# jzbontar/mc-cnn

Measured on AMD Instinct MI355X. Metric: Mega-pixel-disparities/sec (cost-vol+CBCA+SGM) + end-to-end disp ms/pair, higher is better.
Workload: dtype f32; 1 GPU; KITTI 2012 fast, 370x1226 disp_max=228; H=370, W=1226, disp_max=228, feature_channels=64, params=kitti_fast, parallelism=one pair per GPU

## Files before the change

### mc-cnn_amd/csrc/api.hip

```cpp
#include "cbca_common.h"

#include <stdarg.h>
#include <algorithm>
#include <map>
#include <mutex>
#include <vector>

namespace mc {

int fill_nan(float *p, int64_t n, hipStream_t st);
int scale(const float *in, float *out, int64_t n, float s, hipStream_t st);
int transpose(const float *in, float *out, int64_t R, int64_t Cn, int64_t ldin, int64_t ldout, float s, hipStream_t st, int nt = -1);
int fix_border(float *vol, int D, int H, int W, int n, int direction, hipStream_t st);
int argmin_dhw(const float *vol, float *out, int D, int H, int W, int base1, hipStream_t st);
int outlier_detection(const float *d0, const float *d1, float *outlier, int H, int W, int disp_max, hipStream_t st);
int interpolate_occlusion(const float *d0, const float *outlier, float *out, int H, int W, hipStream_t st);
int interpolate_mismatch(const float *d0, const float *outlier, float *out, int H, int W, hipStream_t st);
int subpixel(const float *d0, const float *vol, float *out, int D, int H, int W, int64_t sd, int64_t sp, hipStream_t st);
int median2d(const float *img, float *out, int H, int W, int k, hipStream_t st);
int mean2d(const float *img, const float *kernel, float *out, int H, int W, int ks, float alpha2, hipStream_t st);
int normalize_forward(const float *in, float *norm, float *out, int N, int C, int H, int W, hipStream_t st);
int stereo_join_dhw(const float *fL, const float *fR, float *volL, float *volR, int C, int D, int H, int W, hipStream_t st);
int stereo_join_hwd(const float *fL, const float *fR, float *volL, float *volR, int C, int D, int ds, int H, int W, int n,
                    hipStream_t st);
// ... 17 lines not shown
                  hipStream_t st, bool two_pass = false, float cost_limit = 0);
int cbca_lean2x(const void *packed, const void *plan, size_t plan_bytes, const float *vin, float *vout, int D, int H, int W, int direction,
                int route, hipStream_t st, const CbcaCfg &cfg);
int cbca_lean(const void *packed, const void *plan, size_t plan_bytes, const float *vin, float *vout, int D, int H, int W, int direction,
              int route, hipStream_t st, const CbcaCfg &cfg);
size_t conv3x3_workspace_bytes(int Cin, int Cout);
int conv3x3(const float *in, const float *w, const float *bias, float *out, int N, int Cin, int Cout, int H, int W, int relu,
            void *workspace, hipStream_t st);
size_t fc_workspace_bytes(int C, int n_hidden, int H, int W);
int fc_stack(const float *featL, const float *featR, int C, int H, int W, int D, const float *const *weights,
             const float *const *biases, int n_layers, float *volL, float *volR, void *workspace, hipStream_t st);
size_t sgm_maps_bytes(int H, int W);
int sgm_prep(const float *x0, const float *x1, void *maps, int H, int W, float tau_so, hipStream_t st);
int sgm_contract_violations(const float *vol, int H, int W, int D, unsigned *count, hipStream_t st);
int sgm_sweeps(const float *const C[2], float *const out[2], float *const out2[2], float *const disp[2],
               const int direction[2], int nvol, int H, int W, int D, int ds, const void *maps, float pi1, float pi2,
               float alpha1, float q1, float q2, bool fused, unsigned drop_final, hipStream_t st);

static thread_local char g_err[512] = "";

void set_error(const char *fmt, ...)
{
	va_list ap;
	va_start(ap, fmt);
	vsnprintf(g_err, sizeof(g_err), fmt, ap);
	va_end(ap);
}

int check_launch(const char *what)
{
	const hipError_t e = hipPeekAtLastError();
	if (e != hipSuccess) {
		(void)hipGetLastError();
		set_error("%s: %s", what, hipGetErrorString(e));
		return (int)e;
	}
	return 0;
}

static bool dims_ok(int D, int H, int W) { return D >= 1 && H >= 1 && W >= 1 && (int64_t)D * H * W < ((int64_t)1 << 40); }

static void gaussian_fill(double sigma, float *k)
{
	const int kr = (int)ceil(sigma * 3);
	const int ks = kr * 2 + 1;
	for (int i = 1; i <= ks; ++i) {
		for (int j = 1; j <= ks; ++j) {
			const double y = (i - 1) - kr;
			const double x = (j - 1) - kr;
			k[(size_t)(i - 1) * ks + (j - 1)] = (float)exp(-(x * x + y * y) / (2 * sigma * sigma));
		}
	}
}
struct GaussianK { const float *data; size_t n; };
static int gaussian_cached(double sigma, GaussianK &out)
{
	static std::mutex mu;
	static std::map<double, GaussianK> cache;
	std::lock_guard<std::mutex> lk(mu);
	auto it = cache.find(sigma);
	if (it != cache.end()) { out = it->second; return 0; }
	const int kr = (int)ceil(sigma * 3);
	const int ks = kr * 2 + 1;
	float *k = nullptr;
	const hipError_t e = hipHostMalloc((void **)&k, (size_t)ks * ks * sizeof(float), hipHostMallocDefault);
	if (e != hipSuccess) {
		set_error("gaussian: hipHostMalloc: %s", hipGetErrorString(e));
		return (int)e;
	}
	gaussian_fill(sigma, k);
	out = GaussianK{k, (size_t)ks * ks};
	cache[sigma] = out;
	return 0;
}

static inline size_t align_up(size_t v, size_t a) { return (v + a - 1) / a * a; }

static inline bool packed_dims_ok(int H, int W)
{
	return (int64_t)H * W < ((int64_t)1 << 29) - 4096 && H < (1 << 23) - 64 && W < (1 << 23) - 256;
}

static int cbca_by_arms(const void *packed, const float *vin, float *vout, int D, int H, int W, int direction, int max_arm, hipStream_t st,
                        const CbcaCfg &cfg = CbcaCfg())
{
	if (max_arm >= 0 && max_arm <= 4) return cbca_tiles(packed, vin, vout, D, H, W, direction, 4, -1, st, cfg);
	if (cfg.planned) {
		int rc = cbca_tiles(packed, vin, vout, D, H, W, direction, 13, CR_PLANNED_TILE13, st, cfg);
		if (rc || cfg.lean_two_pass) return rc;
		return cbca_strips(packed, vin, vout, D, H, W, direction, CR_STRIP_IF_LIST, st, cfg);
	}
	int rc = cbca_tiles(packed, vin, vout, D, H, W, direction, 4, CR_TILE4, st, cfg);
	if (rc) return rc;
	if (max_arm < 0 || max_arm <= 13) {
		rc = cbca_tiles(packed, vin, vout, D, H, W, direction, 13, CR_TILE13, st, cfg);
		if (rc) return rc;
	}
	if (cfg.lean) {
		if (!cfg.lean_two_pass) {
			rc = cbca_lean(packed, cfg.plan, cfg.plan_bytes, vin, vout, D, H, W, direction, CR_STRIP, st, cfg);
			if (rc) return rc;
		}
		return cbca_strips(packed, vin, vout, D, H, W, direction, CR_STRIP_IF_NO_LIST, st, cfg);
	}
	return cbca_strips(packed, vin, vout, D, H, W, direction, max_arm > 13 ? CR_STRIP_OR_TILE13 : CR_STRIP, st, cfg);
}

struct Plan {
	int Dp;
	size_t maps, arms, pack, vol, img, gk;
	size_t cplan;
	int nplan;
	size_t total;
};

struct StageCounts { int cbca1, sgm, cbca2; bool active_after; };
static StageCounts stage_counts(const mc_params *p)
{
	StageCounts c;
	bool sm_active = p->sm_terminate != MC_SM_CNN;
	c.cbca1 = (sm_active && p->sm_skip != MC_SKIP_CBCA) ? p->cbca_i1 : 0;
	sm_active = sm_active && p->sm_terminate != MC_SM_CBCA1;
	c.sgm = (sm_active && p->sm_skip != MC_SKIP_SGM) ? p->sgm_i : 0;
	sm_active = sm_active && p->sm_terminate != MC_SM_SGM;
	c.cbca2 = (sm_active && p->sm_skip != MC_SKIP_CBCA) ? p->cbca_i2 : 0;
// ... 41 lines not shown
	{
		for (int i = 0; i < MC_N_STAGES; ++i) out[i] = 0;
		if (!on || ev.empty()) return;
		(void)hipEventSynchronize(ev.back());
		for (size_t i = 1; i < ev.size(); ++i) {
			float ms = 0;
			(void)hipEventElapsedTime(&ms, ev[i - 1], ev[i]);
			if (tag[i] >= 0 && tag[i] < MC_N_STAGES) out[tag[i]] += ms;
		}
		for (auto e : ev) (void)hipEventDestroy(e);
		ev.clear();
	}
};
enum { ST_PREP = MC_STAGE_PREP, ST_JOIN = MC_STAGE_JOIN, ST_CBCA = MC_STAGE_CBCA, ST_LAYOUT = MC_STAGE_LAYOUT,
       ST_SGM = MC_STAGE_SGM, ST_ARGMIN = MC_STAGE_ARGMIN, ST_POST = MC_STAGE_POST };

static int predict_impl(const mc_params *p, const float *x0, const float *x1, const float *featL, const float *featR, int C,
                        const float *rawL, const float *rawR, int D, int H, int W, void *workspace, size_t workspace_bytes,
                        float *volL_out, float *volR_out, float *dispL0_out, float *dispR0_out, float *disp_out, hipStream_t st,
                        StageTimer &tm)
{
	MC_REQUIRE(p && x0 && x1 && disp_out && workspace, "mc_predict: null argument");
	MC_REQUIRE(dims_ok(D, H, W), "mc_predict: bad dims D=%d H=%d W=%d", D, H, W);
	MC_REQUIRE(D <= MC_SGM_MAX_D, "mc_predict: D=%d exceeds %d", D, MC_SGM_MAX_D);
	MC_REQUIRE((featL && featR && C >= 1) || (rawL && rawR), "mc_predict: need features or raw volumes");
	MC_REQUIRE(p->cbca_i1 >= 0 && p->cbca_i2 >= 0 && p->sgm_i >= 0, "mc_predict: negative iteration count");
	MC_REQUIRE(p->median_k % 2 == 1 && p->median_k <= 11, "mc_predict: median_k must be odd and <= 11");
	MC_REQUIRE(p->blur_sigma > 0, "mc_predict: blur_sigma must be > 0");
	MC_REQUIRE(p->sm_terminate >= 0 && p->sm_terminate <= MC_SM_BILATERAL && p->sm_skip >= 0 && p->sm_skip <= MC_SKIP_BILATERAL,
	           "mc_predict: bad sm_terminate / sm_skip");
	const bool from_feat = featL != nullptr;
	if (from_feat) MC_REQUIRE(p->border_n >= 0 && p->border_n < W, "mc_predict: border_n=%d out of range", p->border_n);
	if (from_feat) MC_REQUIRE(C <= MC_JOIN_MAX_C, "mc_predict: C=%d exceeds %d (adcensus.cu:1460)", C, MC_JOIN_MAX_C);
	const Plan pl = make_plan(p, D, H, W);
	MC_REQUIRE(workspace_bytes >= pl.total, "mc_predict: workspace %zu < %zu bytes", workspace_bytes, pl.total);
	MC_REQUIRE((uintptr_t)workspace % 256 == 0, "mc_predict: workspace must be 256-byte aligned");

	const int64_t HW = (int64_t)H * W;
	const int64_t V = (int64_t)D * HW;
	char *w = (char *)workspace;
	void *maps = w; w += pl.maps;
	float *x0c = (float *)w; float *x1c = x0c + 4 * HW; w += pl.arms;
	void *packed = w; w += pl.pack;
	float *bufA[2], *bufB[2];
	bufA[0] = (float *)w; w += pl.vol;
	bufA[1] = (float *)w; w += pl.vol;
	bufB[0] = (float *)w; w += pl.vol;
	bufB[1] = (float *)w; w += pl.vol;
	float *bufC[2];
	bufC[0] = (float *)w; w += pl.vol;
	bufC[1] = (float *)w; w += pl.vol;
	float *img[6];
	for (int i = 0; i < 6; ++i) { img[i] = (float *)w; w += pl.img; }
	float *gk = (float *)w; w += pl.gk;
	void *cplan[2] = {pl.cplan ? (void *)w : nullptr, (pl.cplan && pl.nplan > 1) ? (void *)(w + pl.cplan) : nullptr};
	int cplan_passes[2] = {0, 0};
	bool cplan_listed[2] = {false, false};
	const int Dp = pl.Dp;
	int rc;
#define RUN(call) do { rc = (call); if (rc) return rc; } while (0)

	const int direction[2] = {-1, 1};
	const StageCounts sc = stage_counts(p);
	const int n_cbca1 = sc.cbca1, n_sgm = sc.sgm, n_cbca2 = sc.cbca2;
	bool sm_active = sc.active_after;
	const bool use_cbca = (n_cbca1 + n_cbca2) > 0;
	tm.mark(-1);

	if (n_sgm > 0) RUN(sgm_prep(x0, x1, maps, H, W, p->tau_so, st));
	if (use_cbca) {
		RUN(cross(x0, x0c, H, W, p->L1, p->tau1, st));
		RUN(cross(x1, x1c, H, W, p->L1, p->tau1, st));
		RUN(cbca_pack(x0c, x1c, packed, H, W, st));
	}
	const int cbca_cap = p->L1 - 1;
	tm.mark(ST_PREP);

	const int ds = Dp;
	const float *cur[2];
	auto other = [&](int v) -> float * { return cur[v] == bufA[v] ? bufB[v] : bufA[v]; };
	bool hwd;
	const int nvol = (p->left_only && !p->lr_check && !volR_out && !dispR0_out) ? 1 : 2;
	auto cbca_iterations = [&](int n) -> int {
		const bool packed_ok = cbca_cap <= 254 && packed_dims_ok(H, W);
		for (int v = 0; v < nvol; ++v) {
			const bool planned = packed_ok && cplan[v] && cbca_cap > 4 && cbca_cap <= 13 && cbca_lean_fits(D, H, W, pl.cplan, true);
			if (planned && n > 0 && !cplan_listed[v]) {
				const int rc1 = cbca_classify(packed, cplan[v], pl.cplan, D, H, W, direction[v], CR_STRIP, 0, 0, st, true);
				if (rc1) return rc1;
				cplan_listed[v] = true;
			}
			for (int i = 0; i < n;) {
				float *dst = other(v);
				CbcaCfg cfg;
				cfg.plan = cplan[v];
				cfg.plan_bytes = pl.cplan;
				cfg.planned = planned;
				const bool two = planned && i + 1 < n;
				cfg.lean = cfg.lean_two_pass = two;
				float *mid = two ? bufC[v] : dst;
				for (int half = 0; half < (two ? 2 : 1); ++half) {
					cfg.plan_mode = cplan[v] ? (cplan_passes[v]++ == 0 ? 1 : 2) : 0;
					const float *src = half == 0 ? cur[v] : mid;
					float *to = (two && half == 0) ? mid : dst;
					const int rc2 = packed_ok ? cbca_by_arms(packed, src, to, D, H, W, direction[v], cbca_cap, st, cfg)
					                          : cbca(x0c, x1c, src, to, D, H, W, direction[v], st);
					if (rc2) return rc2;
// ... 72 lines not shown
	MC_REQUIRE(have_disp || !hwd, "mc_predict: an (H,W,D) volume without its arg-min");
	if (!have_disp) {
		for (int v = 0; v < nvol; ++v) RUN(argmin_dhw(cur[v], dispv[v], D, H, W, 0, st));
	}
	float *vout[2] = {volL_out, volR_out};
	for (int v = 0; v < nvol; ++v) {
		if (!vout[v]) continue;
		if (hwd) RUN(transpose(cur[v], vout[v], HW, D, ds, HW, 1.0f, st));
		else RUN(scale(cur[v], vout[v], V, 1.0f, st));
	}
	if (dispL0_out) RUN(scale(dispv[0], dispL0_out, HW, 1.0f, st));
	if (dispR0_out) RUN(scale(dispv[1], dispR0_out, HW, 1.0f, st));
	tm.mark(ST_ARGMIN);

	float *d = dispv[0];
	float *outl = img[4];
	int nfree = 0;
	float *freeimg[3] = {img[2], img[3], img[5]};
	auto next = [&]() -> float * {
		float *r = freeimg[nfree % 3];
		if (r == d) r = freeimg[++nfree % 3];
		++nfree;
		return r;
	};
	if (p->lr_check) {
		RUN(outlier_detection(d, dispv[1], outl, H, W, D, st));
		if (sm_active && p->sm_skip != MC_SKIP_OCCLUSION) {
			float *o = next();
			RUN(interpolate_occlusion(d, outl, o, H, W, st));
			d = o;
		}
		sm_active = sm_active && p->sm_terminate != MC_SM_OCCLUSION;
		if (sm_active && p->sm_skip != MC_SKIP_OCCLUSION) {
			float *o = next();
			RUN(interpolate_mismatch(d, outl, o, H, W, st));
			d = o;
		}
		sm_active = sm_active && p->sm_terminate != MC_SM_MISMATCH;
	}
	if (sm_active && p->sm_skip != MC_SKIP_SUBPIXEL) {
		float *o = next();
		if (hwd) RUN(subpixel(d, cur[0], o, D, H, W, 1, ds, st));
		else RUN(subpixel(d, cur[0], o, D, H, W, HW, 1, st));
		d = o;
	}
	sm_active = sm_active && p->sm_terminate != MC_SM_SUBPIXEL;
	if (sm_active && p->sm_skip != MC_SKIP_MEDIAN) {
		float *o = next();
		RUN(median2d(d, o, H, W, p->median_k, st));
		d = o;
	}
	sm_active = sm_active && p->sm_terminate != MC_SM_MEDIAN;
	if (sm_active && p->sm_skip != MC_SKIP_BILATERAL) {
		GaussianK k;
		RUN(gaussian_cached(p->blur_sigma, k));
		const int ks = 2 * (int)ceil(p->blur_sigma * 3) + 1;
		const hipError_t e = hipMemcpyAsync(gk, k.data, k.n * sizeof(float), hipMemcpyHostToDevice, st);
		if (e != hipSuccess) {
			set_error("mc_predict: kernel upload: %s", hipGetErrorString(e));
			return (int)e;
		}
		RUN(mean2d(d, gk, disp_out, H, W, ks, p->blur_t, st));
	} else {
		RUN(scale(d, disp_out, HW, 1.0f, st));
	}
	tm.mark(ST_POST);
#undef RUN
	return 0;
}

}

using namespace mc;

extern "C" {

int mc_version(void) { return MC_ABI_VERSION; }
const char *mc_last_error(void) { return g_err; }

int mc_fill_nan(float *p, int64_t n, void *stream)
{
	MC_REQUIRE(p || n == 0, "mc_fill_nan: null pointer");
	MC_REQUIRE(n >= 0, "mc_fill_nan: negative size");
	return fill_nan(p, n, as_stream(stream));
}

int mc_stereo_join(const float *featL, const float *featR, float *volL, float *volR, int C, int D, int H, int W, void *stream)
{
	MC_REQUIRE(featL && featR && volL && volR, "mc_stereo_join: null pointer");
	MC_REQUIRE(dims_ok(D, H, W) && C >= 1, "mc_stereo_join: bad dims C=%d D=%d H=%d W=%d", C, D, H, W);
	MC_REQUIRE(C <= MC_JOIN_MAX_C, "mc_stereo_join: C=%d exceeds %d (adcensus.cu:1460)", C, MC_JOIN_MAX_C);
	MC_REQUIRE(D <= 65535, "mc_stereo_join: D too large");
	return stereo_join_dhw(featL, featR, volL, volR, C, D, H, W, as_stream(stream));
}

int mc_ad(const float *x0, const float *x1, float *vol, int D, int H, int W, int direction, void *stream)
{
	MC_REQUIRE(x0 && x1 && vol, "mc_ad: null pointer");
	MC_REQUIRE(dims_ok(D, H, W), "mc_ad: bad dims");
	MC_REQUIRE(direction == -1 || direction == 1, "mc_ad: direction must be -1 or 1");
	MC_REQUIRE(D <= 65535, "mc_ad: D too large");
	return ad_tiled(x0, x1, vol, D, H, W, direction, as_stream(stream));
}

size_t mc_census_scratch_bytes(int Cimg, int H, int W)
{
	if (Cimg < 1 || H < 1 || W < 1) return 0;
	return census_scratch_bytes(Cimg, H, W);
}

int mc_census_ws(const float *x0, const float *x1, float *vol, int Cimg, int D, int H, int W, int direction, void *scratch,
                 size_t scratch_bytes, void *stream)
{
	MC_REQUIRE(x0 && x1 && vol && scratch, "mc_census_ws: null pointer");
	MC_REQUIRE(dims_ok(D, H, W) && Cimg >= 1 && D <= 65535, "mc_census_ws: bad dims");
// ... 369 lines not shown
```

### mc-cnn_amd/csrc/post.hip

```cpp
#include "mc_common.h"

namespace mc {


__global__ void __launch_bounds__(256) fill_nan_kernel(float *__restrict__ p, int64_t n)
{
	const float nanv = __builtin_nanf("");
	for (int64_t i = (int64_t)blockIdx.x * blockDim.x + threadIdx.x; i < n; i += (int64_t)gridDim.x * blockDim.x) p[i] = nanv;
}

__global__ void __launch_bounds__(256) scale_kernel(const float *__restrict__ in, float *__restrict__ out, int64_t n, float s)
{
	for (int64_t i = (int64_t)blockIdx.x * blockDim.x + threadIdx.x; i < n; i += (int64_t)gridDim.x * blockDim.x) out[i] = in[i] * s;
}
typedef float f4v_t __attribute__((ext_vector_type(4)));
__global__ void __launch_bounds__(256) scale4_kernel(const f4v_t *__restrict__ in, f4v_t *__restrict__ out, int64_t n4, float s)
{
	const int64_t i = (int64_t)blockIdx.x * 256 + threadIdx.x;
	if (i < n4) out[i] = in[i] * s;
}

template <bool NT>
__global__ void __launch_bounds__(256) transpose_kernel(const float *__restrict__ in, float *__restrict__ out, int64_t R,
                                                        int64_t Cn, int64_t ldin, int64_t ldout, float s)
// ... 198 lines not shown
	__shared__ int carry[256];
	__shared__ int first_valid;
	const int y = blockIdx.x, t = threadIdx.x;
	const int64_t row = (int64_t)y * W;
	const int seg = (W + 255) / 256;
	const int xa = t * seg, xb = min(W, xa + seg);
	if (t == 0) first_valid = W;
	int last = -1;
	for (int x = xa; x < xb; ++x)
		if (outlier[row + x] == 0) last = x;
	carry[t] = last;
	__syncthreads();
	if (last >= 0) {
		int f = -1;
		for (int x = xa; x < xb; ++x)
			if (outlier[row + x] == 0) { f = x; break; }
		atomicMin(&first_valid, f);
	}
	for (int off = 1; off < 256; off <<= 1) {
		const int o = t >= off ? carry[t - off] : -1;
		__syncthreads();
		carry[t] = max(carry[t], o);
		__syncthreads();
	}
	int lv = t > 0 ? carry[t - 1] : -1;
	const int fv = first_valid;
	for (int x = xa; x < xb; ++x) {
		const int64_t id = row + x;
		const float o = outlier[id];
		if (o == 0) lv = x;
		float r = d0[id];
		if (o == 1) {
			if (lv >= 0) r = d0[row + lv];
			else if (fv < W) r = d0[row + fv];
		}
		out[id] = r;
	}
}

int interpolate_occlusion(const float *d0, const float *outlier, float *out, int H, int W, hipStream_t st)
{
	hipLaunchKernelGGL(interp_occ_rows_kernel, dim3(H), dim3(256), 0, st, d0, outlier, out, W);
	return check_launch("interpolate_occlusion");
}

template <int K> __device__ __forceinline__ void ray_rank_step(float v, int inb, int &less, int &eq)
{
	const float ov = __uint_as_float(__builtin_amdgcn_update_dpp(0u, __float_as_uint(v), 0x120 + K, 0xf, 0xf, false));
	const int oin = __builtin_amdgcn_update_dpp(0, inb, 0x120 + K, 0xf, 0xf, false);
	less += (oin && ov < v) ? 1 : 0;
	eq += (oin && ov == v) ? 1 : 0;
}

#define MC_MIS_NU 4
__global__ void __launch_bounds__(256) interp_mis_rays_kernel(const float *__restrict__ d0, const float *__restrict__ outlier,
                                                              float *__restrict__ out, int size, int H, int W)
{
	const int t = blockIdx.x * blockDim.x + threadIdx.x;
	const int id = t >> 4;
	const int ray = (int)(threadIdx.x & 15);
	if (id >= size) return;
	const bool mis = outlier[id] == 2;
	if (!mis) {
		if (ray == 0) out[id] = d0[id];
		return;
	}
	const int hx[16] = {0, -1, -2, -2, -2, -2, -2, -1, 0, 1, 2, 2, 2, 2, 2, 1};
	const int hy[16] = {2, 2, 2, 1, 0, -1, -2, -2, -2, -2, -2, -1, 0, 1, 2, 2};
	const int x = id % W, y = id / W;
	const int sx = hx[ray], sy = hy[ray];
	const __amdgpu_buffer_rsrc_t ro = __builtin_amdgcn_make_buffer_rsrc((void *)outlier, 0, size * 4, 0x00020000);
	const __amdgpu_buffer_rsrc_t rd = __builtin_amdgcn_make_buffer_rsrc((void *)d0, 0, size * 4, 0x00020000);
	int X2 = 2 * x, Y2 = 2 * y;
	constexpr unsigned OOB = 0x80000000u;
	unsigned stop = OOB;
	for (bool go = true; go;) {
		unsigned off[MC_MIS_NU], o[MC_MIS_NU];
#pragma unroll
		for (int i = 0; i < MC_MIS_NU; ++i) {
			X2 += sx;
			Y2 += sy;
			const int xi = (X2 + 1 + (X2 >> 31)) >> 1;
			const int yi = (Y2 + 1 + (Y2 >> 31)) >> 1;
			const bool in = (unsigned)yi < (unsigned)H && (unsigned)xi < (unsigned)W;
			off[i] = in ? (__umul24((unsigned)yi, (unsigned)W) + (unsigned)xi) * 4u : OOB;
			o[i] = __builtin_amdgcn_raw_buffer_load_b32(ro, off[i], 0, 0);
		}
#pragma unroll
		for (int i = MC_MIS_NU - 1; i >= 0; --i) {
			const bool hit = __uint_as_float(o[i]) != 2.0f;
			stop = hit ? off[i] : stop;
			go = hit ? false : go;
		}
	}
	const int inb = stop != OOB ? 1 : 0;
	const float v = __uint_as_float(__builtin_amdgcn_raw_buffer_load_b32(rd, stop, 0, 0));
	int less = 0, eq = inb;
	ray_rank_step<1>(v, inb, less, eq); ray_rank_step<2>(v, inb, less, eq); ray_rank_step<3>(v, inb, less, eq);
	ray_rank_step<4>(v, inb, less, eq); ray_rank_step<5>(v, inb, less, eq); ray_rank_step<6>(v, inb, less, eq);
	ray_rank_step<7>(v, inb, less, eq); ray_rank_step<8>(v, inb, less, eq); ray_rank_step<9>(v, inb, less, eq);
	ray_rank_step<10>(v, inb, less, eq); ray_rank_step<11>(v, inb, less, eq); ray_rank_step<12>(v, inb, less, eq);
	ray_rank_step<13>(v, inb, less, eq); ray_rank_step<14>(v, inb, less, eq); ray_rank_step<15>(v, inb, less, eq);
	const uint64_t bal = __ballot(inb != 0);
	const int n = __builtin_popcount((unsigned)((bal >> ((threadIdx.x & 48))) & 0xffffu));
	if (n == 0) {
		if (ray == 0) out[id] = d0[id];
		return;
	}
	const int want = n / 2;
	if (inb && less <= want && want < less + eq) out[id] = v;
}

int interpolate_mismatch(const float *d0, const float *outlier, float *out, int H, int W, hipStream_t st)
{
	const int64_t size = (int64_t)H * W;
	MC_REQUIRE(size * 16 < ((int64_t)1 << 31), "interpolate_mismatch: %dx%d pixels x 16 rays do not fit a 32-bit index", H, W);
	MC_REQUIRE(H < (1 << 24) && W < (1 << 24), "interpolate_mismatch: %dx%d: a side beyond the 24-bit row / column arithmetic of the ray walk", H, W);
	hipLaunchKernelGGL(interp_mis_rays_kernel, dim3(cdiv(size * 16, 256)), dim3(256), 0, st, d0, outlier, out, (int)size, H, W);
	return check_launch("interpolate_mismatch");
}

__global__ void __launch_bounds__(256) subpixel_kernel(const float *__restrict__ d0, const float *__restrict__ c2,
                                                       float *__restrict__ out, int64_t size, int64_t sd, int64_t sp, int disp_max)
{
	const int64_t id = (int64_t)blockIdx.x * blockDim.x + threadIdx.x;
	if (id >= size) return;
	const int d = (int)d0[id];
	float res = (float)d;
	if (1 <= d && d < disp_max - 1) {
		const float cn = c2[(d - 1) * sd + id * sp];
		const float cz = c2[d * sd + id * sp];
		const float cp = c2[(d + 1) * sd + id * sp];
		const float denom = 2 * (cp + cn - 2 * cz);
		if ((double)denom > 1e-5) {
			res = (float)((double)d - fmin(1.0, fmax(-1.0, (double)((cp - cn) / denom))));
		}
	}
	out[id] = res;
}

int subpixel(const float *d0, const float *vol, float *out, int D, int H, int W, int64_t sd, int64_t sp, hipStream_t st)
{
	const int64_t size = (int64_t)H * W;
	hipLaunchKernelGGL(subpixel_kernel, dim3(cdiv(size, 256)), dim3(256), 0, st, d0, vol, out, size, sd, sp, D);
	return check_launch("subpixel_enchancement");
}

__device__ __forceinline__ void cswap(float &a, float &b)
{
	const float lo = fminf(a, b), hi = fmaxf(a, b);
	a = lo;
	b = hi;
}

template <int N>
__device__ __forceinline__ float median_forgetful(const float (&v)[N])
{
	constexpr int M0 = N / 2 + 2;
	float w[M0];
#pragma unroll
	for (int i = 0; i < M0; ++i) w[i] = v[i];
	int next = M0;
#pragma unroll
	for (int m = M0; m > 3; --m) {
#pragma unroll
		for (int i = 0; i < m / 2; ++i) cswap(w[i], w[m - 1 - i]);
#pragma unroll
		for (int i = 1; i < (m + 1) / 2; ++i) cswap(w[0], w[i]);
#pragma unroll
		for (int i = m / 2; i < m - 1; ++i) cswap(w[i], w[m - 1]);
		w[0] = v[next < N ? next : N - 1];
		++next;
	}
	cswap(w[0], w[1]);
	cswap(w[1], w[2]);
	cswap(w[0], w[1]);
	return w[1];
}

template <int KR>
__global__ void __launch_bounds__(256) median_kernel(const float *__restrict__ img, float *__restrict__ out, int H, int W)
{
	constexpr int K = 2 * KR + 1;
	constexpr int TW = 64 + 2 * KR, TH = 4 + 2 * KR;
	__shared__ float tile[TH][TW + 1];
	const int bx = blockIdx.x * 64, by = blockIdx.y * 4;
	for (int i = threadIdx.x; i < TH * TW; i += 256) {
		const int ty = i / TW, tx = i % TW;
		const int gx = bx + tx - KR, gy = by + ty - KR;
		tile[ty][tx] = (gx >= 0 && gx < W && gy >= 0 && gy < H) ? img[(int64_t)gy * W + gx] : 0.0f;
	}
	__syncthreads();
	const int lx = threadIdx.x & 63, ly = threadIdx.x >> 6;
	const int x = bx + lx, y = by + ly;
	if (x >= W || y >= H) return;
	const int xa = max(0, x - KR), xb = min(W - 1, x + KR), ya = max(0, y - KR), yb = min(H - 1, y + KR);
	const int n = (xb - xa + 1) * (yb - ya + 1);
	if constexpr (KR == 1 || KR == 2) {
		if (n == K * K) {
			float v[K * K];
#pragma unroll
			for (int i = 0; i < K * K; ++i) v[i] = tile[ly + i % K][lx + i / K];
			out[(int64_t)y * W + x] = median_forgetful<K * K>(v);
			return;
		}
	}
	const int want = n / 2;
	float res = 0;
	for (int i = 0; i < K * K; ++i) {
		const int ix = x - KR + i / K, iy = y - KR + i % K;
		if (ix < xa || ix > xb || iy < ya || iy > yb) continue;
		const float vi = tile[iy - by + KR][ix - bx + KR];
		int less = 0, eq = 0;
		for (int yy = ya; yy <= yb; ++yy) {
			for (int xx = xa; xx <= xb; ++xx) {
				const float vj = tile[yy - by + KR][xx - bx + KR];
				less += vj < vi ? 1 : 0;
				eq += vj == vi ? 1 : 0;
			}
		}
		if (less <= want && want < less + eq) {
			res = vi;
			break;
		}
	}
	out[(int64_t)y * W + x] = res;
}

int median2d(const float *img, float *out, int H, int W, int k, hipStream_t st)
{
	const dim3 grid(cdiv(W, 64), cdiv(H, 4)), block(256);
	switch (k / 2) {
	case 0: hipLaunchKernelGGL(median_kernel<0>, grid, block, 0, st, img, out, H, W); break;
	case 1: hipLaunchKernelGGL(median_kernel<1>, grid, block, 0, st, img, out, H, W); break;
	case 2: hipLaunchKernelGGL(median_kernel<2>, grid, block, 0, st, img, out, H, W); break;
	case 3: hipLaunchKernelGGL(median_kernel<3>, grid, block, 0, st, img, out, H, W); break;
	case 4: hipLaunchKernelGGL(median_kernel<4>, grid, block, 0, st, img, out, H, W); break;
	default: hipLaunchKernelGGL(median_kernel<5>, grid, block, 0, st, img, out, H, W); break;
	}
	return check_launch("median2d");
}

constexpr int M2_OY = 2;
constexpr int M2_TR = 4;
__global__ void __launch_bounds__(64 * M2_TR) mean2d_kernel(const float *__restrict__ img, const float *__restrict__ kernel,
                                                            float *__restrict__ out, int H, int W, int kr, float alpha2)
{
	extern __shared__ __attribute__((aligned(16))) float smem[];
	constexpr int NT = 64 * M2_TR;
	const int ks = 2 * kr + 1;
	const int TW = 64 + 2 * kr, TH = M2_TR * M2_OY + 2 * kr;
	const int TS = TW + 1;
	const int WS = ks + 2 * (M2_OY - 1);
	float *tile = smem;
	float *wts = smem + TH * TS;
	const int bx = blockIdx.x * 64, by = blockIdx.y * (M2_TR * M2_OY);
	const float FAR = 1e30f;
	for (int i = threadIdx.x; i < TH * TW; i += NT) {
// ... 198 lines not shown
```

### mc-cnn_amd/csrc/sgm.hip

```cpp
#include "mc_common.h"

#define MC_SGM_VOL_AUX 2
#define MC_SGM_ST_AUX MC_SGM_VOL_AUX

namespace mc {

constexpr int SGM_PADW = 520;

struct SgmPassArgs {
	const float *C[2];
	const float *accin[2];
	const float *accin2[2];
	float *out[2];
	float *out2[2];
	float *disp[2];
	int drop_out[2];
	int direction[2];
	int nvol;
	int H, W, D, ds;
	const uint8_t *cls0;
	int64_t cls_plane;
	const uint8_t *win;
	int Wm;
	float P1[3], P2[3], P1a[3];
};

__device__ __forceinline__ int cls_of(float v, float tau) { return v < tau ? 0 : (v > tau ? 2 : 1); }

__global__ void __launch_bounds__(256) sgm_prep_kernel(const float *__restrict__ x0, const float *__restrict__ x1,
                                                       uint8_t *__restrict__ cls0, uint8_t *__restrict__ win,
                                                       int H, int W, int Wm, int64_t cls_plane, float tau_so)
{
	const int64_t id = (int64_t)blockIdx.x * blockDim.x + threadIdx.x;
	const int64_t total = (int64_t)4 * H * Wm;
	if (id >= total) return;
	const int i = (int)(id % Wm);
	const int y = (int)((id / Wm) % H);
	const int r = (int)(id / ((int64_t)Wm * H));
	const int dx = r == 0 ? 1 : (r == 1 ? -1 : 0);
	const int dy = r == 2 ? 1 : (r == 3 ? -1 : 0);
	const bool yok = (y - dy >= 0) && (y - dy < H);

	if (i < W) {
		const int x = i;
		int c = 1;
		if (yok && x - dx >= 0 && x - dx < W) {
			c = cls_of(fabsf(x0[y * W + x] - x0[(y - dy) * W + x - dx]), tau_so);
		}
		cls0[(int64_t)r * cls_plane + (int64_t)y * W + x] = (uint8_t)c;
	}
	const int s = i - SGM_PADW;
	unsigned asc = 0, desc = 0;
#pragma unroll
	for (int k = 0; k < 4; ++k) {
		const int xx = s + k;
		float D2 = 10.0f;
		if (yok && xx >= 0 && xx < W && xx - dx >= 0 && xx - dx < W) {
			D2 = fabsf(x1[y * W + xx] - x1[(y - dy) * W + xx - dx]);
		}
		const unsigned c = (unsigned)cls_of(D2, tau_so);
		asc |= c << (2 * k);
		desc |= c << (2 * (3 - k));
	}
	win[((int64_t)(0 * 4 + r) * H + y) * Wm + i] = (uint8_t)asc;
	win[((int64_t)(1 * 4 + r) * H + y) * Wm + i] = (uint8_t)desc;
}

typedef unsigned uint4v __attribute__((ext_vector_type(4)));

template <int VPL, int NACC>
struct StepData {
	float c[VPL];
	float a[NACC > 0 ? VPL : 1];
	float a2[NACC > 1 ? VPL : 1];
	unsigned pk;
	unsigned a0;
};


__device__ __forceinline__ float vmin2(float a, float b)
{
	float r;
	asm("v_min_f32 %0, %1, %2" : "=v"(r) : "v"(a), "v"(b));
	return r;
}
__device__ __forceinline__ float vmin3(float a, float b, float c)
{
	float r;
	asm("v_min3_f32 %0, %1, %2, %3" : "=v"(r) : "v"(a), "v"(b), "v"(c));
	return r;
}
__device__ __forceinline__ float wave_min_q(float v)
{
	float r;
	asm volatile("s_nop 1\n\tv_min_f32_dpp %1, %1, %1 quad_perm:[1,0,3,2] row_mask:0xf bank_mask:0xf\n\t"
	             "s_nop 1\n\tv_min_f32_dpp %1, %1, %1 quad_perm:[2,3,0,1] row_mask:0xf bank_mask:0xf\n\t"
	             "s_nop 1\n\tv_min_f32_dpp %1, %1, %1 row_half_mirror row_mask:0xf bank_mask:0xf\n\t"
	             "s_nop 1\n\tv_min_f32_dpp %1, %1, %1 row_mirror row_mask:0xf bank_mask:0xf\n\t"
	             "s_nop 1\n\tv_min_f32_dpp %1, %1, %1 row_bcast:15 row_mask:0xa bank_mask:0xf\n\t"
	             "s_nop 1\n\tv_min_f32_dpp %1, %1, %1 row_bcast:31 row_mask:0xc bank_mask:0xf\n\t"
	             "s_nop 0\n\tv_readlane_b32 %0, %1, 63"
	             : "=s"(r), "+v"(v));
	return r;
}

__device__ __forceinline__ __amdgpu_buffer_rsrc_t pixel_rsrc(const float *base, int64_t elem_off, int bytes)
{
	return __builtin_amdgcn_make_buffer_rsrc((void *)(base + elem_off), 0, bytes, 0x00020000);
}

template <int DIRN, int VPL, int MODE, bool ARGMIN, bool VEC, int U, bool DUAL, bool FAR>
__device__ __forceinline__ void sgm_line(const SgmPassArgs &A, int wave)
{
	constexpr int NACC = MODE == 0 ? 0 : (MODE == 3 ? 2 : 1);
	const int lane = threadIdx.x & 63;
	const int H = A.H, W = A.W, D = A.D, ds = A.ds, Wm = A.Wm;
	const int nlines = DIRN <= 1 ? H : W;
	const int nsteps = DIRN <= 1 ? W : H;
// ... 230 lines not shown
}

template <int DIRN, int VPL, int MODE, bool ARGMIN, bool VEC, int U, bool DUAL, bool FAR>
__global__ void __launch_bounds__(256) sgm_pass_kernel(const SgmPassArgs A)
{
	sgm_line<DIRN, VPL, MODE, ARGMIN, VEC, U, DUAL, FAR>(A, __builtin_amdgcn_readfirstlane((int)((blockIdx.x * blockDim.x + threadIdx.x) >> 6)));
}


__global__ void __launch_bounds__(256) sgm_contract_kernel(const float *__restrict__ vol, int64_t pixels, int D, unsigned *__restrict__ count)
{
	const int64_t p = (int64_t)blockIdx.x * blockDim.x + threadIdx.x;
	bool bad = false;
	if (p < pixels) {
		const float *v = vol + p * D;
		bad = !(fabsf(v[0]) < __builtin_inff());
		bool seen_nan = false;
		for (int d = 0; d < D; ++d) {
			const bool isn = v[d] != v[d];
			bad = bad || (seen_nan && !isn);
			seen_nan = seen_nan || isn;
		}
	}
	const unsigned long long b = __ballot(bad);
	if ((threadIdx.x & 63) == 0 && b) atomicAdd(count, (unsigned)__builtin_popcountll(b));
}

int sgm_contract_violations(const float *vol, int H, int W, int D, unsigned *count, hipStream_t st)
{
	const int64_t pixels = (int64_t)H * W;
	hipError_t e = hipMemsetAsync(count, 0, sizeof(unsigned), st);
	if (e != hipSuccess) {
		set_error("mc_sgm2_contract_violations: hipMemsetAsync: %s", hipGetErrorString(e));
		return (int)e;
	}
	hipLaunchKernelGGL(sgm_contract_kernel, dim3(cdiv(pixels, 256)), dim3(256), 0, st, vol, pixels, D, count);
	return check_launch("sgm_contract");
}

size_t sgm_maps_bytes(int H, int W)
{
	const size_t Wm = (size_t)W + 2 * SGM_PADW;
	const size_t plane = ((size_t)H * W + 3 + 4) / 4 * 4;
	size_t b = 4 * plane + (size_t)8 * H * Wm;
	return (b + 255) & ~(size_t)255;
}

int sgm_prep(const float *x0, const float *x1, void *maps, int H, int W, float tau_so, hipStream_t st)
{
	const int Wm = W + 2 * SGM_PADW;
	const size_t plane = ((size_t)H * W + 3 + 4) / 4 * 4;
	uint8_t *cls0 = (uint8_t *)maps;
	uint8_t *win = cls0 + 4 * plane;
	const int64_t total = (int64_t)4 * H * Wm;
	hipLaunchKernelGGL(sgm_prep_kernel, dim3(cdiv(total, 256)), dim3(256), 0, st, x0, x1, cls0, win, H, W, Wm, (int64_t)plane,
	                   tau_so);
	return check_launch("sgm_prep");
}

constexpr int SGM_U_H = 8, SGM_U_UP = 16;
constexpr int SGM_U_DOWN = 16;

template <int DIRN, int MODE, bool ARGMIN, bool DUAL>
static void launch_pass(const SgmPassArgs &A, bool vec, hipStream_t st)
{
	const int nlines = DIRN <= 1 ? A.H : A.W;
	const int waves = A.nvol * nlines * (DUAL ? 2 : 1);
	const dim3 grid(cdiv(waves, 4)), block(256);
	const int U = DIRN == 2 ? SGM_U_DOWN : (DIRN == 3 ? SGM_U_UP : SGM_U_H);
	constexpr bool SCALAR = MODE == 1;
#define MC_SGM_GO(VPL_, VEC_, U_) \
	hipLaunchKernelGGL((sgm_pass_kernel<DIRN, VPL_, MODE, ARGMIN, VEC_, U_, DUAL, false>), grid, block, 0, st, A)
#define MC_SGM_GO_FAR(VPL_, VEC_, U_) \
	hipLaunchKernelGGL((sgm_pass_kernel<DIRN, VPL_, MODE, ARGMIN, VEC_, U_, DUAL, true>), grid, block, 0, st, A)
	const bool far = (int64_t)A.H * A.W * A.ds * 4 >= ((int64_t)1 << 31);
	if (!vec) {
		if constexpr (SCALAR) {
			if (far) { if (A.D <= 256) MC_SGM_GO_FAR(4, false, 4); else MC_SGM_GO_FAR(8, false, 2); }
			else { if (A.D <= 256) MC_SGM_GO(4, false, 4); else MC_SGM_GO(8, false, 2); }
		}
	} else if (far) {
		if (A.D <= 256) MC_SGM_GO_FAR(4, true, 4); else MC_SGM_GO_FAR(8, true, 4);
	} else if (A.D <= 256) {
		if (U == 16) MC_SGM_GO(4, true, 16); else if (U == 8) MC_SGM_GO(4, true, 8); else MC_SGM_GO(4, true, 4);
	} else {
		if (U >= 8) MC_SGM_GO(8, true, 8); else MC_SGM_GO(8, true, 4);
	}
#undef MC_SGM_GO_FAR
#undef MC_SGM_GO
}


int sgm_sweeps(const float *const C[2], float *const out[2], float *const out2[2], float *const disp[2],
               const int direction[2], int nvol, int H, int W, int D, int ds, const void *maps, float pi1, float pi2,
               float alpha1, float q1, float q2, bool fused, unsigned drop_final, hipStream_t st)
{
	MC_REQUIRE((int64_t)H * W < ((int64_t)1 << 29) && (int64_t)W * ds * 4 < ((int64_t)1 << 31), "sgm: image %dx%d (pixel stride %d) exceeds the sweeps' 32-bit line arithmetic", H, W, ds);
	SgmPassArgs A;
	for (int v = 0; v < 2; ++v) {
		const int k = v < nvol ? v : 0;
		A.C[v] = C[k];
		A.accin[v] = out[k];
		A.accin2[v] = out2 ? out2[k] : nullptr;
		A.out[v] = out[k];
		A.out2[v] = out2 ? out2[k] : nullptr;
		A.disp[v] = disp ? disp[k] : nullptr;
		A.direction[v] = direction[k];
		A.drop_out[v] = 0;
	}
// ... 35 lines not shown
```

Measured before the change: 81180 MPix-disp/s.

## Cache gaussian kernel on device, batch mismatch rays, pack SGM prep, pad median borders

The Gaussian blur kernel is now uploaded once per device and cached, which removes a per-call host-to-device copy from the stream. The mismatch-interpolation ray walk uses precomputed step deltas and growing batch sizes, with a bound on the remaining in-image steps. SGM prep now has each thread produce four window bytes, reusing seven shared edge classes and writing packed dwords. The median filter handles borders with ±inf padding so edge pixels use the fast sorting network. These are several unrelated micro-optimizations on small stages, and they add some risk around the per-device cache lifetime and border-correctness logic.

```diff
diff --git a/mc-cnn_amd/csrc/api.hip b/mc-cnn_amd/csrc/api.hip
--- a/mc-cnn_amd/csrc/api.hip
+++ b/mc-cnn_amd/csrc/api.hip
@@ -93,25 +93,36 @@
 		}
 	}
 }
-struct GaussianK { const float *data; size_t n; };
-static int gaussian_cached(double sigma, GaussianK &out)
+static int gaussian_device(double sigma, const float *&out)
 {
 	static std::mutex mu;
-	static std::map<double, GaussianK> cache;
+	static std::map<std::pair<int, double>, const float *> cache;
+	int dev = 0;
+	hipError_t e = hipGetDevice(&dev);
+	if (e != hipSuccess) {
+		set_error("gaussian: hipGetDevice: %s", hipGetErrorString(e));
+		return (int)e;
+	}
 	std::lock_guard<std::mutex> lk(mu);
-	auto it = cache.find(sigma);
+	const auto key = std::make_pair(dev, sigma);
+	auto it = cache.find(key);
 	if (it != cache.end()) { out = it->second; return 0; }
 	const int kr = (int)ceil(sigma * 3);
 	const int ks = kr * 2 + 1;
-	float *k = nullptr;
-	const hipError_t e = hipHostMalloc((void **)&k, (size_t)ks * ks * sizeof(float), hipHostMallocDefault);
+	std::vector<float> k((size_t)ks * ks);
+	gaussian_fill(sigma, k.data());
+	float *d = nullptr;
+	e = hipMalloc((void **)&d, k.size() * sizeof(float));
+	if (e == hipSuccess) {
+		e = hipMemcpy(d, k.data(), k.size() * sizeof(float), hipMemcpyHostToDevice);
+		if (e != hipSuccess) (void)hipFree(d);
+	}
 	if (e != hipSuccess) {
-		set_error("gaussian: hipHostMalloc: %s", hipGetErrorString(e));
+		(void)hipGetLastError();
+		set_error("gaussian: device copy: %s", hipGetErrorString(e));
 		return (int)e;
 	}
-	gaussian_fill(sigma, k);
-	out = GaussianK{k, (size_t)ks * ks};
-	cache[sigma] = out;
+	cache[key] = out = d;
 	return 0;
 }
 
@@ -259,7 +270,7 @@
 	bufC[1] = (float *)w; w += pl.vol;
 	float *img[6];
 	for (int i = 0; i < 6; ++i) { img[i] = (float *)w; w += pl.img; }
-	float *gk = (float *)w; w += pl.gk;
+	w += pl.gk;
 	void *cplan[2] = {pl.cplan ? (void *)w : nullptr, (pl.cplan && pl.nplan > 1) ? (void *)(w + pl.cplan) : nullptr};
 	int cplan_passes[2] = {0, 0};
 	bool cplan_listed[2] = {false, false};
@@ -438,15 +449,10 @@
 	}
 	sm_active = sm_active && p->sm_terminate != MC_SM_MEDIAN;
 	if (sm_active && p->sm_skip != MC_SKIP_BILATERAL) {
-		GaussianK k;
-		RUN(gaussian_cached(p->blur_sigma, k));
+		const float *k = nullptr;
+		RUN(gaussian_device(p->blur_sigma, k));
 		const int ks = 2 * (int)ceil(p->blur_sigma * 3) + 1;
-		const hipError_t e = hipMemcpyAsync(gk, k.data, k.n * sizeof(float), hipMemcpyHostToDevice, st);
-		if (e != hipSuccess) {
-			set_error("mc_predict: kernel upload: %s", hipGetErrorString(e));
-			return (int)e;
-		}
-		RUN(mean2d(d, gk, disp_out, H, W, ks, p->blur_t, st));
+		RUN(mean2d(d, k, disp_out, H, W, ks, p->blur_t, st));
 	} else {
 		RUN(scale(d, disp_out, HW, 1.0f, st));
 	}
diff --git a/mc-cnn_amd/csrc/post.hip b/mc-cnn_amd/csrc/post.hip
--- a/mc-cnn_amd/csrc/post.hip
+++ b/mc-cnn_amd/csrc/post.hip
@@ -274,7 +274,34 @@
 	eq += (oin && ov == v) ? 1 : 0;
 }
 
-#define MC_MIS_NU 4
+__device__ __forceinline__ int ray_steps_inside(int s, int x, int n)
+{
+	return s == 0 ? 0x3fffffff : (s == -1 ? 2 * x : (s == 1 ? 2 * (n - 1 - x) : (s == -2 ? x : n - 1 - x)));
+}
+
+constexpr unsigned MIS_OOB = 0x80000000u;
+constexpr unsigned MIS_NONE = 0xffffffffu;
+
+template <int N>
+__device__ __forceinline__ unsigned ray_batch(const __amdgpu_buffer_rsrc_t ro, unsigned &off, int &left, unsigned d_odd, unsigned d_even)
+{
+	unsigned o[N], at[N];
+#pragma unroll
+	for (int i = 0; i < N; ++i) {
+		off += (i & 1) ? d_even : d_odd;
+		at[i] = i < left ? off : MIS_OOB;
+		o[i] = __builtin_amdgcn_raw_buffer_load_b32(ro, at[i], 0, 0);
+	}
+	left -= N;
+	unsigned stop = MIS_NONE;
+#pragma unroll
+	for (int i = N - 1; i >= 0; --i) stop = __uint_as_float(o[i]) != 2.0f ? at[i] : stop;
+	return stop;
+}
+
+#ifndef MC_MIS_CAP
+#define MC_MIS_CAP 32
+#endif
 __global__ void __launch_bounds__(256) interp_mis_rays_kernel(const float *__restrict__ d0, const float *__restrict__ outlier,
                                                               float *__restrict__ out, int size, int H, int W)
 {
@@ -293,29 +320,15 @@
 	const int sx = hx[ray], sy = hy[ray];
 	const __amdgpu_buffer_rsrc_t ro = __builtin_amdgcn_make_buffer_rsrc((void *)outlier, 0, size * 4, 0x00020000);
 	const __amdgpu_buffer_rsrc_t rd = __builtin_amdgcn_make_buffer_rsrc((void *)d0, 0, size * 4, 0x00020000);
-	int X2 = 2 * x, Y2 = 2 * y;
-	constexpr unsigned OOB = 0x80000000u;
-	unsigned stop = OOB;
-	for (bool go = true; go;) {
-		unsigned off[MC_MIS_NU], o[MC_MIS_NU];
-#pragma unroll
-		for (int i = 0; i < MC_MIS_NU; ++i) {
-			X2 += sx;
-			Y2 += sy;
-			const int xi = (X2 + 1 + (X2 >> 31)) >> 1;
-			const int yi = (Y2 + 1 + (Y2 >> 31)) >> 1;
-			const bool in = (unsigned)yi < (unsigned)H && (unsigned)xi < (unsigned)W;
-			off[i] = in ? (__umul24((unsigned)yi, (unsigned)W) + (unsigned)xi) * 4u : OOB;
-			o[i] = __builtin_amdgcn_raw_buffer_load_b32(ro, off[i], 0, 0);
-		}
-#pragma unroll
-		for (int i = MC_MIS_NU - 1; i >= 0; --i) {
-			const bool hit = __uint_as_float(o[i]) != 2.0f;
-			stop = hit ? off[i] : stop;
-			go = hit ? false : go;
-		}
-	}
-	const int inb = stop != OOB ? 1 : 0;
+	const int ox = (sx + 1) >> 1, oy = (sy + 1) >> 1;
+	const unsigned d_odd = (unsigned)(oy * W + ox) * 4u, d_even = (unsigned)((sy - oy) * W + (sx - ox)) * 4u;
+	int left = min(ray_steps_inside(sx, x, W), ray_steps_inside(sy, y, H));
+	unsigned off = (unsigned)id * 4u;
+	unsigned stop = ray_batch<4>(ro, off, left, d_odd, d_even);
+	if (stop == MIS_NONE) stop = ray_batch<8>(ro, off, left, d_odd, d_even);
+	if (stop == MIS_NONE) stop = ray_batch<16>(ro, off, left, d_odd, d_even);
+	while (stop == MIS_NONE) stop = ray_batch<MC_MIS_CAP>(ro, off, left, d_odd, d_even);
+	const int inb = stop != MIS_OOB ? 1 : 0;
 	const float v = __uint_as_float(__builtin_amdgcn_raw_buffer_load_b32(rd, stop, 0, 0));
 	int less = 0, eq = inb;
 	ray_rank_step<1>(v, inb, less, eq); ray_rank_step<2>(v, inb, less, eq); ray_rank_step<3>(v, inb, less, eq);
@@ -419,13 +432,23 @@
 	const int xa = max(0, x - KR), xb = min(W - 1, x + KR), ya = max(0, y - KR), yb = min(H - 1, y + KR);
 	const int n = (xb - xa + 1) * (yb - ya + 1);
 	if constexpr (KR == 1 || KR == 2) {
-		if (n == K * K) {
-			float v[K * K];
-#pragma unroll
-			for (int i = 0; i < K * K; ++i) v[i] = tile[ly + i % K][lx + i / K];
-			out[(int64_t)y * W + x] = median_forgetful<K * K>(v);
-			return;
-		}
+		constexpr int T = K * K;
+		float v[T];
+		if (n == T) {
+#pragma unroll
+			for (int i = 0; i < T; ++i) v[i] = tile[ly + i % K][lx + i / K];
+		} else {
+			int pads = T / 2 - n / 2;
+#pragma unroll
+			for (int i = 0; i < T; ++i) {
+				const int ix = x - KR + i / K, iy = y - KR + i % K;
+				const bool in = ix >= xa && ix <= xb && iy >= ya && iy <= yb;
+				v[i] = in ? tile[ly + i % K][lx + i / K] : (pads > 0 ? -INFINITY : INFINITY);
+				pads -= in ? 0 : 1;
+			}
+		}
+		out[(int64_t)y * W + x] = median_forgetful<T>(v);
+		return;
 	}
 	const int want = n / 2;
 	float res = 0;
diff --git a/mc-cnn_amd/csrc/sgm.hip b/mc-cnn_amd/csrc/sgm.hip
--- a/mc-cnn_amd/csrc/sgm.hip
+++ b/mc-cnn_amd/csrc/sgm.hip
@@ -27,43 +27,74 @@
 
 __device__ __forceinline__ int cls_of(float v, float tau) { return v < tau ? 0 : (v > tau ? 2 : 1); }
 
+__device__ __forceinline__ int edge_cls(const float *__restrict__ img, int W, int y, int x, int dx, int dy, bool yok, float tau_so,
+                                        int none)
+{
+	if (!(yok && x >= 0 && x < W && x - dx >= 0 && x - dx < W)) return none;
+	return cls_of(fabsf(img[y * W + x] - img[(y - dy) * W + x - dx]), tau_so);
+}
+
 __global__ void __launch_bounds__(256) sgm_prep_kernel(const float *__restrict__ x0, const float *__restrict__ x1,
                                                        uint8_t *__restrict__ cls0, uint8_t *__restrict__ win,
-                                                       int H, int W, int Wm, int64_t cls_plane, float tau_so)
-{
-	const int64_t id = (int64_t)blockIdx.x * blockDim.x + threadIdx.x;
-	const int64_t total = (int64_t)4 * H * Wm;
-	if (id >= total) return;
-	const int i = (int)(id % Wm);
-	const int y = (int)((id / Wm) % H);
-	const int r = (int)(id / ((int64_t)Wm * H));
-	const int dx = r == 0 ? 1 : (r == 1 ? -1 : 0);
-	const int dy = r == 2 ? 1 : (r == 3 ? -1 : 0);
-	const bool yok = (y - dy >= 0) && (y - dy < H);
-
-	if (i < W) {
-		const int x = i;
-		int c = 1;
-		if (yok && x - dx >= 0 && x - dx < W) {
-			c = cls_of(fabsf(x0[y * W + x] - x0[(y - dy) * W + x - dx]), tau_so);
-		}
-		cls0[(int64_t)r * cls_plane + (int64_t)y * W + x] = (uint8_t)c;
-	}
-	const int s = i - SGM_PADW;
-	unsigned asc = 0, desc = 0;
-#pragma unroll
-	for (int k = 0; k < 4; ++k) {
-		const int xx = s + k;
-		float D2 = 10.0f;
-		if (yok && xx >= 0 && xx < W && xx - dx >= 0 && xx - dx < W) {
-			D2 = fabsf(x1[y * W + xx] - x1[(y - dy) * W + xx - dx]);
-		}
-		const unsigned c = (unsigned)cls_of(D2, tau_so);
-		asc |= c << (2 * k);
-		desc |= c << (2 * (3 - k));
-	}
-	win[((int64_t)(0 * 4 + r) * H + y) * Wm + i] = (uint8_t)asc;
-	win[((int64_t)(1 * 4 + r) * H + y) * Wm + i] = (uint8_t)desc;
+                                                       int H, int W, int Wm, int64_t cls_plane, float tau_so, int dword_ok)
+{
+	const int64_t q = (int64_t)blockIdx.x * blockDim.x + threadIdx.x;
+	const int64_t rows = (int64_t)4 * H, total = rows * Wm;
+	if (q * 4 >= total) return;
+	const int c_out = cls_of(10.0f, tau_so);
+	unsigned asc[4], desc[4];
+	{
+		const int64_t ry = q * 4 / Wm;
+		const int i0 = (int)(q * 4 - ry * Wm);
+		if (i0 + 3 < Wm) {
+			const int r = (int)(ry / H), y = (int)(ry % H);
+			const int dx = r == 0 ? 1 : (r == 1 ? -1 : 0);
+			const int dy = r == 2 ? 1 : (r == 3 ? -1 : 0);
+			const bool yok = (y - dy >= 0) && (y - dy < H);
+			const int s = i0 - SGM_PADW;
+			unsigned c[7];
+			if (yok && s + 6 >= 0 && s < W) {
+#pragma unroll
+				for (int j = 0; j < 7; ++j) c[j] = (unsigned)edge_cls(x1, W, y, s + j, dx, dy, yok, tau_so, c_out);
+			} else {
+#pragma unroll
+				for (int j = 0; j < 7; ++j) c[j] = (unsigned)c_out;
+			}
+#pragma unroll
+			for (int b = 0; b < 4; ++b) {
+				asc[b] = c[b] | c[b + 1] << 2 | c[b + 2] << 4 | c[b + 3] << 6;
+				desc[b] = c[b] << 6 | c[b + 1] << 4 | c[b + 2] << 2 | c[b + 3];
+				const int x = i0 + b;
+				if (x < W) cls0[(int64_t)r * cls_plane + (int64_t)y * W + x] = (uint8_t)edge_cls(x0, W, y, x, dx, dy, yok, tau_so, 1);
+			}
+		} else {
+			for (int b = 0; b < 4; ++b) {
+				const int64_t f = q * 4 + b, ryb = f / Wm;
+				const int i = (int)(f - ryb * Wm);
+				const int r = (int)(ryb / H), y = (int)(ryb % H);
+				const int dx = r == 0 ? 1 : (r == 1 ? -1 : 0);
+				const int dy = r == 2 ? 1 : (r == 3 ? -1 : 0);
+				const bool yok = (y - dy >= 0) && (y - dy < H);
+				asc[b] = desc[b] = 0;
+				for (int k = 0; k < 4; ++k) {
+					const unsigned c = (unsigned)edge_cls(x1, W, y, i - SGM_PADW + k, dx, dy, yok, tau_so, c_out);
+					asc[b] |= c << (2 * k);
+					desc[b] |= c << (2 * (3 - k));
+				}
+				if (i < W) cls0[(int64_t)r * cls_plane + (int64_t)y * W + i] = (uint8_t)edge_cls(x0, W, y, i, dx, dy, yok, tau_so, 1);
+			}
+		}
+	}
+	uint8_t *wa = win + q * 4, *wd = win + total + q * 4;
+	if (dword_ok) {
+		*(unsigned *)wa = asc[0] | asc[1] << 8 | asc[2] << 16 | asc[3] << 24;
+		*(unsigned *)wd = desc[0] | desc[1] << 8 | desc[2] << 16 | desc[3] << 24;
+	} else {
+		for (int b = 0; b < 4; ++b) {
+			wa[b] = (uint8_t)asc[b];
+			wd[b] = (uint8_t)desc[b];
+		}
+	}
 }
 
 typedef unsigned uint4v __attribute__((ext_vector_type(4)));
@@ -400,9 +431,10 @@
 	const size_t plane = ((size_t)H * W + 3 + 4) / 4 * 4;
 	uint8_t *cls0 = (uint8_t *)maps;
 	uint8_t *win = cls0 + 4 * plane;
-	const int64_t total = (int64_t)4 * H * Wm;
-	hipLaunchKernelGGL(sgm_prep_kernel, dim3(cdiv(total, 256)), dim3(256), 0, st, x0, x1, cls0, win, H, W, Wm, (int64_t)plane,
-	                   tau_so);
+	const int64_t groups = (int64_t)H * Wm;
+	const int dword_ok = ((uintptr_t)win & 3) == 0;
+	hipLaunchKernelGGL(sgm_prep_kernel, dim3(cdiv(groups, 256)), dim3(256), 0, st, x0, x1, cls0, win, H, W, Wm, (int64_t)plane,
+	                   tau_so, dword_ok);
 	return check_launch("sgm_prep");
 }
 
```

After: 82510 MPix-disp/s (median of 4 runs). About the same (+1.6%).
